# rustic-rs/rustic_core

Measured on AMD Instinct MI355X. Metric: CDC chunking GiB/s device-resident, 1/2/4/8 MI355X; bit-exact cut points vs ref, higher is better.
Workload: dtype u8

## Files before the change

rustic_core_amd/csrc/rcdc_ingest.cpp:

```cpp
#include <hip/hip_runtime.h>

#include <sys/random.h>

#include <algorithm>
#include <atomic>
#include <chrono>
#include <cmath>
#include <condition_variable>
#include <cstdio>
#include <cstdlib>
#include <cstring>
#include <deque>
#include <functional>
#include <memory>
#include <mutex>
#include <string>
#include <thread>
#include <unordered_map>
#include <unordered_set>
#include <vector>

#include "../../include/rcdc.h"
#include "rcdc_host.h"
#include "rcdc_ingest_steps.h"
// ... 33 lines not shown
    }
};

template <typename H, hipError_t (*Destroy)(H)>
struct HipOwner {
    H h = nullptr;
    HipOwner() = default;
    HipOwner(HipOwner &&o) noexcept : h(o.h) { o.h = nullptr; }
    ~HipOwner() { reset(); }
    void reset() {
        if (h) (void)Destroy(h);
        h = nullptr;
    }
    operator H() const { return h; }
};
using Stream = HipOwner<hipStream_t, hipStreamDestroy>;
struct Event : HipOwner<hipEvent_t, hipEventDestroy> {
    hipError_t create() { return hipEventCreateWithFlags(&h, hipEventDisableTiming); }
};

hipError_t ing_alloc(rcdc_ingest *g, void **p, uint64_t n, bool pinned);
hipError_t ing_free(void *p);

template <typename T>
struct IngBuf {
    T *p = nullptr;
    uint64_t cap = 0;
    bool pinned = false;
    IngBuf() = default;
    IngBuf(const IngBuf &) = delete;
    ~IngBuf() { (void)release(); }
    operator T *() const { return p; }
    hipError_t release() {
        T *q = p;
        p = nullptr, cap = 0;
        return q ? ing_free(q) : hipSuccess;
    }
    hipError_t alloc(rcdc_ingest *g, uint64_t n, bool pin) {
        pinned = pin;
        const hipError_t e = ing_alloc(g, (void **)&p, n * sizeof(T), pin);
        cap = e == hipSuccess ? n : 0;
        return e;
    }
    bool ensure(rcdc_ingest *g, uint64_t need, uint64_t grown, const char *what);
};

struct StreamSt {
    uint64_t handle = 0, tag = 0, hint = 0;
    uint64_t fed = 0;
    uint32_t open_pieces = 0;
    bool closed = false, aborted = false;
    int cslot = -1;
    uint64_t base = 0;
    uint64_t carry_len = 0;
    std::vector<uint8_t> hcarry;
    std::vector<uint64_t> cuts;
    std::vector<uint8_t> ids;
    uint32_t nnew = 0;
};

struct FileEnt {
    uint64_t tag = 0;
    uint64_t off = 0;
    uint64_t res = 0;
    uint64_t len = 0;
    bool done = false;
    bool cancelled = false;
    bool final = false;
    std::shared_ptr<StreamSt> st;
};

struct Unit {
    uint64_t tag = 0;
    std::shared_ptr<StreamSt> st;
    bool final = true, aborted = false;
    uint64_t base = 0;
    uint64_t carry = 0;
    uint64_t off = 0, len = 0;
    uint64_t fresh = 0;
    std::vector<std::pair<uint64_t, uint64_t>> segs;
    std::vector<std::pair<const uint8_t *, uint64_t>> host;
};

enum SlotState { kFree = 0, kOpen, kClosed, kSubmitted };

struct InSlot {
    IngBuf<uint8_t> host;
    uint64_t used = 0;
    uint32_t open_res = 0;
    SlotState state = kFree;
    std::vector<FileEnt> files;
    Event h2d;
    bool h2d_pending = false;
    std::atomic<int> host_jobs{0};
    std::atomic<bool> h2d_issued{false};
    uint64_t close_seq = 0;
    bool has_stream = false;
    double t_first = 0;
    void reset(SlotState to) {
        state = to;
        used = 0;
        files.clear();
        has_stream = false;
        t_first = 0;
    }
};

struct OutSlot {
    IngBuf<uint8_t> host;
    std::atomic<int> packs_left{0};
    bool busy = false;
};

struct D2HDone {
    Event fin;
    std::atomic<bool> issued{false};
};

struct Batch {
    uint64_t index = 0;
    uint32_t pslot = 0;
    InSlot *in = nullptr;
    std::vector<FileEnt> files;
    std::vector<Unit> units;
    std::vector<uint64_t> cuts;
    std::vector<uint32_t> ncuts;
    std::vector<uint64_t> c_off, c_len;
    std::vector<const uint8_t *> c_host;
    std::vector<std::vector<uint8_t>> gathers;
    std::vector<uint8_t> ids;
    std::vector<uint32_t> short_idx;
    std::vector<uint64_t> seal_off, seal_len, ulen;
    std::atomic<int> long_jobs{0};
    std::vector<rcdc_pack_blob> blobs;
    std::vector<std::pair<uint32_t, uint32_t>> grp;
    size_t open_from = 0;
    std::vector<rcdc_pack> packs;
    uint64_t total = 0;
    std::vector<uint32_t> boffs;
    OutSlot *out = nullptr;
    std::vector<std::pair<steps::D2HRange, std::shared_ptr<D2HDone>>> d2h;
};

struct PlanDel {
    void operator()(rcdc_plan *p) const { rcdc_plan_destroy(p); }
};
struct PSlot {
    std::unique_ptr<rcdc_plan, PlanDel> plan;
    IngBuf<uint8_t> arena;
    IngBuf<uint8_t> staging;
    IngBuf<uint64_t> d_refs;
    IngBuf<uint64_t> h_refs;
    IngBuf<uint8_t> d_dig;
    Stream s_ids;
    Event ev_ids;
    Event ev_sealed;
    Event ev_retired;
    bool busy = false;
};

struct PackJob {
    OutSlot *out = nullptr;
    uint64_t off = 0, size = 0, seq = 0, batch = 0;
    uint32_t header_len = 0;
    std::vector<rcdc_ingest_blob> blobs;
    uint8_t id[32];
};

long long env_num(const char *name, long long dflt) {
    const char *e = getenv(name);
    return e ? strtoll(e, nullptr, 10) : dflt;
}
struct Knobs {
    size_t tail_batches = (size_t)env_num("RCDC_INGEST_TAIL_BATCHES", 2);
    uint64_t d2h_group = (uint64_t)env_num("RCDC_INGEST_D2H_GROUP", 256ll << 20);
    bool tail_single = env_num("RCDC_INGEST_TAIL_SINGLE", 1) != 0;
    uint32_t id_threads = (uint32_t)env_num("RCDC_INGEST_ID_THREADS", 0);
    bool poll = env_num("RCDC_INGEST_POLL", 1) != 0;
    uint32_t kcopy = (uint32_t)std::max(env_num("RCDC_INGEST_KCOPY", 0), 0ll);
    uint64_t copy_piece = (uint64_t)std::max(env_num("RCDC_INGEST_COPY_PIECE", 64ll << 20), 1ll << 20);
    int prof = getenv("RCDC_INGEST_PROF") ? (int)std::max(env_num("RCDC_INGEST_PROF", 0), 1ll) : 0;
    uint32_t fail_alloc = (uint32_t)std::max(env_num("RCDC_INGEST_FAIL_ALLOC", 0), 0ll);
    bool alloc_log = getenv("RCDC_ALLOC_LOG") != nullptr;
};

}

struct rcdc_index {
    static constexpr int kShards = 64;
    struct Shard {
        std::mutex mu;
        std::unordered_set<Id32, Id32Hash> set;
    };
    Shard sh[kShards];
    bool insert(const Id32 &id) {
        Shard &s = sh[id.b[31] & (kShards - 1)];
        std::lock_guard<std::mutex> lk(s.mu);
        return s.set.insert(id).second;
    }
    uint64_t size() {
        uint64_t n = 0;
        for (auto &s : sh) {
            std::lock_guard<std::mutex> lk(s.mu);
            n += s.set.size();
        }
        return n;
    }
};

struct rcdc_ingest {
    rcdc_ctx *ctx = nullptr;
    rcdc_ingest_config cfg{};
    rcdc_ingest_pack_fn pack_cb = nullptr;
    rcdc_ingest_file_fn file_cb = nullptr;
    void *user = nullptr;
    int device = 0;
    int level = 0;
    bool compress = true, verify = true;
    uint64_t batch_cap = 0, long_chunk = 0;
    Knobs knobs;
    uint32_t depth = 4, nin = 4, nout = 4, nthreads = 8;
    PackSizer sizer{};
    std::mutex mu;
    std::condition_variable cv_slot;
    std::vector<std::unique_ptr<InSlot>> in;
    InSlot *open = nullptr;
    std::deque<InSlot *> ready;
    std::vector<PSlot> ps;
    IngBuf<uint8_t> frames;
    IngBuf<uint8_t> d_packs;
    IngBuf<uint8_t> carry[2];
    int carry_cur = 0;
    std::vector<rcdc_pack_blob> carry_blobs;
    Stream s_in, s_comp, s_out;
    Event ev_comp, ev_out, ev_back;
    std::vector<std::unique_ptr<OutSlot>> outs;
    std::deque<std::unique_ptr<Batch>> submitted;
    std::deque<std::unique_ptr<Batch>> inflight;
    bool front_done = false;
    uint64_t nclosed = 0;
    Stream s_back;
    uint64_t nbatches = 0, next_seq = 0;
    rcdc_index *idx = nullptr;
    std::unique_ptr<rcdc_index> own_idx;
    uint64_t max_chunk = 0;
    uint64_t asm_base = 0, asm_cap = 0;
    IngBuf<uint8_t> carry_pool;
    std::vector<int> free_cslots;
    std::unordered_map<uint64_t, std::shared_ptr<StreamSt>> streams;
    uint64_t next_stream = 1;
    uint32_t closing_streams = 0;
    std::deque<InSlot *> closed_q;
    double pack_t0 = 0;
    double pack_max_age = 300, slot_max_age = 1;
    uint32_t nalloc = 0;
    std::thread worker, back, waiter, feeder;
    struct CopyJob {
        uint8_t *dst;
        const uint8_t *src;
        uint64_t len, done;
        InSlot *in;
        Event after;
        std::shared_ptr<D2HDone> fin;
    };
    std::deque<CopyJob> h2d_q;
    std::mutex d2h_mu;
    std::deque<CopyJob> d2h_q;
    std::shared_ptr<D2HDone> last_d2h;
    int submitting = 0;
    std::vector<std::thread> pool;
    std::mutex pool_mu;
    std::condition_variable pool_cv;
    std::deque<std::function<void()>> jobs;
    std::deque<std::function<void()>> ujobs;
    uint32_t running_packs = 0;
    std::mutex wait_mu;
    std::condition_variable wait_cv;
    struct WaitItem {
        std::shared_ptr<D2HDone> done;
        uint64_t batch;
        std::vector<std::shared_ptr<PackJob>> jobs;
    };
    std::deque<WaitItem> wait_q;
    std::mutex cb_mu;
    std::atomic<bool> stop{false};
    bool finishing = false, finished = false;
    std::atomic<int> packs_pending{0};
    std::condition_variable cv_done;
    rcdc_status err = RCDC_OK;
    std::string err_msg;
    rcdc_ingest_stats st{};
    double t_first = 0;
    std::vector<std::vector<double>> tl;
    std::vector<double> tl_d2h, tl_ids;
};

namespace {

using Ing = rcdc_ingest;

void set_err(Ing *g, rcdc_status s, const std::string &m) {
    std::lock_guard<std::mutex> lk(g->mu);
    if (!g->err) {
        g->err = s;
        g->err_msg = m;
    }
    g->cv_slot.notify_all();
    g->cv_done.notify_all();
}

// ... 177 lines not shown
            std::vector<uint8_t> dig(32 * grp.size());
            for (auto &pj : grp) {
                ptrs.push_back(pj->out->host + pj->off);
                lens.push_back(pj->size);
            }
            hash_group(ptrs.data(), lens.data(), (uint32_t)grp.size(), dig.data(), mb);
            for (size_t i = 0; i < grp.size(); i++) {
                memcpy(grp[i]->id, dig.data() + 32 * i, 32);
                deliver(g, grp[i]);
            }
        });
    }
}

void waiter_main(Ing *g) {
    (void)hipSetDevice(g->device);
    for (;;) {
        Ing::WaitItem w;
        {
            std::unique_lock<std::mutex> lk(g->wait_mu);
            g->wait_cv.wait(lk, [&] { return g->stop || !g->wait_q.empty(); });
            if (g->wait_q.empty()) return;
            w = std::move(g->wait_q.front());
            g->wait_q.pop_front();
        }
        while (!w.done->issued.load() && !g->err && !g->stop)
            std::this_thread::sleep_for(std::chrono::microseconds(50));
        if (!w.done->issued.load()) continue;
        if (wait_event(g, w.done->fin) != hipSuccess) {
            set_err(g, RCDC_ERR_INTERNAL, "pack copy-back failed");
            continue;
        }
        if (g->knobs.prof) {
            std::lock_guard<std::mutex> lk(g->cb_mu);
            if (g->tl_d2h.size() <= w.batch) g->tl_d2h.resize(w.batch + 1, 0);
            g->tl_d2h[w.batch] = now_s() - g->t_first;
        }
        bool is_last;
        {
            std::lock_guard<std::mutex> lk(g->mu);
            is_last = g->front_done && g->inflight.size() <= 2;
            if (!is_last && g->finishing && g->ready.size() + g->nbatches <= w.batch + 4)
                is_last = true;
        }
        hash_packs(g, std::move(w.jobs), is_last);
    }
}

void mark(Ing *g, uint64_t b, double t) {
    if (!g->knobs.prof) return;
    std::lock_guard<std::mutex> lk(g->cb_mu);
    if (g->tl.size() <= b) g->tl.resize(b + 1);
    g->tl[b].push_back(t - g->t_first);
}

bool submit_ready(Ing *g) {
    for (;;) {
        InSlot *in = nullptr;
        uint32_t ps = 0;
        std::unique_ptr<Batch> B;
        {
            std::lock_guard<std::mutex> lk(g->mu);
            if (g->ready.empty()) return true;
            for (ps = 0; ps < g->depth && g->ps[ps].busy; ps++) {
            }
            if (ps == g->depth) return true;
            in = g->ready.front();
            g->ready.pop_front();
            g->submitting++;
            g->ps[ps].busy = true;
            B = std::make_unique<Batch>();
            B->index = g->nbatches++;
            if (g->t_first == 0) g->t_first = now_s();
        }
        B->pslot = ps;
        B->in = in;
        B->files = in->files;
        mark(g, B->index, now_s());
        PSlot &P = g->ps[ps];
        const uint64_t used = in->used;
        const uint64_t need = round_up(used, 256) + 512;
        if (!P.arena.ensure(g, need, grow8(need), "arena")) return false;
        in->h2d_issued = false;
        g->h2d_q.push_back({P.arena, in->host, used, 0, in, {}, nullptr});
        std::lock_guard<std::mutex> lk(g->mu);
        g->submitted.push_back(std::move(B));
        g->submitting--;
        g->cv_slot.notify_all();
    }
}

void reap_inputs(Ing *g);
void close_open_locked(Ing *g);

struct CopyLane {
    std::deque<Event> inflight;
    std::vector<Event> free_ev;
    hipError_t create() {
        free_ev.resize(4);
        for (Event &e : free_ev)
            if (hipError_t r = e.create()) return r;
        return hipSuccess;
    }
};

template <typename Done>
bool pump(Ing *g, hipStream_t s, std::deque<Ing::CopyJob> &q, std::mutex *mu, hipMemcpyKind kind,
          CopyLane &L, Done on_done) {
    while (!L.inflight.empty() && hipEventQuery(L.inflight.front()) == hipSuccess) {
        L.free_ev.push_back(std::move(L.inflight.front()));
        L.inflight.pop_front();
    }
    std::unique_lock<std::mutex> lq;
    if (mu) lq = std::unique_lock<std::mutex>(*mu);
    while (!q.empty() && L.inflight.size() < 2 && !L.free_ev.empty()) {
        Ing::CopyJob &J = q.front();
        if (J.after) {
            ING_HIP(g, hipStreamWaitEvent(s, J.after, 0));
            J.after.reset();
        }
        const uint64_t n = std::min(g->knobs.copy_piece, J.len - J.done);
        if (n) {
            if (g->knobs.kcopy)
                ING_HIP(g, launch_stream_copy(J.dst + J.done, J.src + J.done, (n + 15) & ~15ull,
                                              g->knobs.kcopy, s));
            else
                ING_HIP(g, hipMemcpyAsync(J.dst + J.done, J.src + J.done, n, kind, s));
            ING_HIP(g, hipEventRecord(L.free_ev.back(), s));
            L.inflight.push_back(std::move(L.free_ev.back()));
            L.free_ev.pop_back();
            J.done += n;
        }
        if (J.done == J.len) {
            if (!on_done(J)) return false;
            q.pop_front();
        }
    }
    return true;
}

bool pump_h2d(Ing *g, CopyLane &L) {
    return pump(g, g->s_in, g->h2d_q, nullptr, hipMemcpyHostToDevice, L, [g](Ing::CopyJob &J) {
        ING_HIP(g, hipEventRecord(J.in->h2d, g->s_in));
        J.in->h2d_issued = true;
        std::lock_guard<std::mutex> lk(g->mu);
        g->cv_slot.notify_all();
        return true;
    });
}

bool pump_d2h(Ing *g, CopyLane &L) {
    return pump(g, g->s_out, g->d2h_q, &g->d2h_mu, hipMemcpyDeviceToHost, L, [g](Ing::CopyJob &J) {
        ING_HIP(g, hipEventRecord(g->ev_out, g->s_out));
        ING_HIP(g, hipEventRecord(J.fin->fin, g->s_out));
        J.fin->issued.store(true);
        return true;
    });
}

void feeder_main(Ing *g) {
    (void)hipSetDevice(g->device);
    CopyLane in, out;
    if (in.create() != hipSuccess || out.create() != hipSuccess) {
        set_err(g, RCDC_ERR_INTERNAL, "feeder events");
        return;
    }
    struct Drain {
        Ing *g;
        ~Drain() {
            (void)hipStreamSynchronize(g->s_in);
            (void)hipStreamSynchronize(g->s_out);
        }
    } drain{g};
    for (;;) {
        reap_inputs(g);
        if (!submit_ready(g) || !pump_h2d(g, in) || !pump_d2h(g, out)) return;
        bool d2h_idle;
        {
            std::lock_guard<std::mutex> lq(g->d2h_mu);
            d2h_idle = g->d2h_q.empty();
        }
        std::unique_lock<std::mutex> lk(g->mu);
        if (g->open && !g->open->files.empty() && now_s() - g->open->t_first >= g->slot_max_age)
            close_open_locked(g);
        if (g->err || (g->finished && g->h2d_q.empty() && d2h_idle)) return;
        g->cv_slot.wait_for(lk, std::chrono::microseconds(g->h2d_q.empty() && d2h_idle ? 200 : 50));
    }
}

const uint8_t *unit_host(const Unit &u, uint64_t rel, uint64_t len) {
    uint64_t at = 0;
    for (const auto &h : u.host) {
        if (rel >= at && rel + len <= at + h.second) return h.first + (rel - at);
        at += h.second;
    }
    return nullptr;
}

void unit_gather(const Unit &u, uint64_t rel, uint64_t len, uint8_t *dst) {
    uint64_t at = 0;
    for (const auto &h : u.host) {
        const uint64_t a = std::max(rel, at), e = std::min(rel + len, at + h.second);
        if (a < e) memcpy(dst + (a - rel), h.first + (a - at), e - a);
        at += h.second;
    }
}

bool build_units(Ing *g, Batch *B, std::vector<rcdc_copy_ref> &cr, uint64_t *asm_used) {
    InSlot *in = B->in;
    std::unordered_map<StreamSt *, size_t> unit_of;
    for (const FileEnt &f : B->files) {
        if (f.cancelled) continue;
        if (!f.st) {
            Unit u;
            u.tag = f.tag;
            u.off = f.off;
            u.len = u.fresh = f.len;
            u.segs.push_back({f.off, f.len});
            B->units.push_back(std::move(u));
            continue;
        }
        auto it = unit_of.find(f.st.get());
        if (it == unit_of.end()) {
            Unit u;
            u.st = f.st;
            u.tag = f.st->tag;
            u.final = false;
            u.base = f.st->base;
            u.carry = f.st->carry_len;
            it = unit_of.emplace(f.st.get(), B->units.size()).first;
            B->units.push_back(std::move(u));
        }
        Unit &u = B->units[it->second];
        if (f.final) {
            u.final = true;
            u.aborted = f.st->aborted;
        }
        if (!f.len) continue;
        if (!u.segs.empty() && u.segs.back().first + u.segs.back().second == f.off)
            u.segs.back().second += f.len;
        else
            u.segs.push_back({f.off, f.len});
        u.fresh += f.len;
    }
    uint64_t ao = 0;
    for (Unit &u : B->units) {
        if (!u.st) {
            u.host.push_back({in->host + u.off, u.len});
            continue;
        }
        u.len = u.carry + u.fresh;
        if (!u.carry && u.segs.size() <= 1) {
            u.off = u.segs.empty() ? 0 : u.segs[0].first;
            if (u.fresh) u.host.push_back({in->host + u.off, u.fresh});
            continue;
        }
        u.off = g->asm_base + ao;
        uint64_t o = u.off;
        if (u.carry) {
            rcdc_copy_ref c{};
            c.in_off = (uint64_t)u.st->cslot * g->max_chunk;
            c.out_off = o;
            c.len = u.carry;
            c.src = 1;
            cr.push_back(c);
            u.host.push_back({u.st->hcarry.data(), u.carry});
            o += u.carry;
        }
        for (const auto &sg : u.segs) {
            rcdc_copy_ref c{};
            c.in_off = sg.first;
            c.out_off = o;
            c.len = sg.second;
            c.src = 0;
            cr.push_back(c);
            u.host.push_back({in->host + sg.first, sg.second});
            o += sg.second;
        }
        ao = round_up(ao + u.len, 256);
        if (ao > g->asm_cap) {
            set_err(g, RCDC_ERR_INTERNAL, "ingest: assembly region overflow");
            return false;
        }
    }
    *asm_used = ao;
    return true;
}


bool a_wait_h2d(Ing *g, Batch *B) {
    InSlot *in = B->in;
    {
        std::unique_lock<std::mutex> lk(g->mu);
        while (!in->h2d_issued && !g->err) g->cv_slot.wait_for(lk, std::chrono::microseconds(100));
        if (g->err) return false;
    }
    ING_HIP(g, hipStreamWaitEvent(g->s_comp, in->h2d, 0));
    if (g->knobs.prof > 1) mark(g, B->index, now_s());
    return true;
}

bool a_gather_units(Ing *g, Batch *B, PSlot &P, uint64_t *arena_len) {
    std::vector<rcdc_copy_ref> gcr;
    uint64_t asm_used = 0;
    if (!build_units(g, B, gcr, &asm_used)) return false;
    if (!gcr.empty()) {
        const void *gsrc[2] = {P.arena, g->carry_pool};
        ING_ST(g, rcdc_copy_ranges(g->ctx, gsrc, 2, gcr.data(), (uint32_t)gcr.size(), P.arena,
                                   g->s_comp),
               "stream gather");
    }
    *arena_len = std::max(round_up(B->in->used, 256) + 256,
                          asm_used ? g->asm_base + asm_used + 256 : 0);
    return true;
}

bool a_chunk(Ing *g, Batch *B, PSlot &P, uint64_t arena_len, std::vector<uint64_t> &cuts,
             std::vector<uint64_t> &counts) {
    const uint32_t nf = (uint32_t)B->units.size();
    std::vector<uint64_t> offs(nf), lens(nf);
    uint64_t ubytes = 0;
    for (uint32_t i = 0; i < nf; i++) {
        offs[i] = B->units[i].off;
        lens[i] = B->units[i].len;
        ubytes += lens[i];
    }
    if (!P.plan) {
        rcdc_plan *pl = nullptr;
        ING_ST(g, rcdc_plan_create(g->ctx, offs.data(), lens.data(), nf, arena_len, &pl), "plan");
        P.plan.reset(pl);
    } else {
        ING_ST(g, plan_relayout(P.plan.get(), offs.data(), lens.data(), nf, arena_len, g->s_comp),
               "plan");
    }
    if (g->knobs.prof > 1) mark(g, B->index, now_s());
    ING_ST(g, rcdc_plan_run(P.plan.get(), P.arena, g->s_comp), "chunk");
    if (g->knobs.prof > 1) {
        (void)hipEventSynchronize(B->in->h2d);
        mark(g, B->index, now_s());
    }
    const uint64_t cap = (uint64_t)nf + ubytes / 4096 + 16;
    cuts.assign(std::max<uint64_t>(cap, 1), 0);
    counts.assign(std::max<uint32_t>(nf, 1), 0);
    rcdc_status rs = rcdc_plan_results(P.plan.get(), cuts.data(), cuts.size(), counts.data());
    if (rs == RCDC_ERR_CAPACITY) {
        uint64_t tot = 0;
        for (uint32_t i = 0; i < nf; i++) tot += counts[i];
        cuts.resize(tot);
        rs = rcdc_plan_results(P.plan.get(), cuts.data(), cuts.size(), counts.data());
    }
    ING_ST(g, rs, "chunk results");
    mark(g, B->index, now_s());
    return true;
}

steps::CutLists a_cut_lists(Ing *g, Batch *B, const std::vector<uint64_t> &cuts,
                            const std::vector<uint64_t> &counts) {
    std::vector<steps::UnitView> uv;
    for (const Unit &u : B->units)
// ... 432 lines not shown

void b_post_packs(Ing *g, Batch *B) {
    std::vector<std::shared_ptr<PackJob>> jobs;
    for (size_t j = 0; j < B->grp.size(); j++) {
        auto pj = std::make_shared<PackJob>();
        pj->out = B->out;
        pj->off = B->packs[j].out_off;
        pj->size = B->packs[j].size;
        pj->header_len = B->packs[j].header_len;
        pj->seq = g->next_seq++;
        pj->batch = B->index;
        for (uint32_t i = B->grp[j].first; i < B->grp[j].first + B->grp[j].second; i++) {
            rcdc_ingest_blob e{};
            memcpy(e.id, B->blobs[i].id, 32);
            e.offset = B->boffs[i];
            e.length = B->blobs[i].len;
            e.uncompressed_length = B->blobs[i].uncompressed_len;
            e.type = B->blobs[i].type;
            pj->blobs.push_back(e);
        }
        jobs.push_back(pj);
    }
    B->out->packs_left += (int)jobs.size();
    g->packs_pending += (int)jobs.size();
    {
        std::lock_guard<std::mutex> lk(g->mu);
        g->st.packs += jobs.size();
        g->st.pack_bytes += B->total;
    }
    {
        std::lock_guard<std::mutex> lk(g->wait_mu);
        for (auto &d : B->d2h)
            g->wait_q.push_back({d.second, B->index,
                                 std::vector<std::shared_ptr<PackJob>>(
                                     jobs.begin() + d.first.first, jobs.begin() + d.first.last)});
    }
    g->wait_cv.notify_one();
}

bool stage_b(Ing *g, Batch *B, bool finalize) {
    const bool has_slot = B->pslot != kNoSlot;
    PSlot &P = g->ps[has_slot ? B->pslot : 0];
    mark(g, B->index, now_s());
    if (has_slot) {
        ING_HIP(g, wait_event(g, P.ev_ids));
        ING_HIP(g, hipStreamWaitEvent(g->s_back, P.ev_sealed, 0));
    }
    mark(g, B->index, now_s());
    if (!b_read_ids(g, B, P)) return false;
    std::vector<uint8_t> is_new;
    const size_t nnew = b_dedup(g, B, is_new);
    b_file_results(g, B, is_new);
    const double tnow = now_s();
    const bool carried = !g->carry_blobs.empty();
    const bool aged = carried && tnow - g->pack_t0 >= g->pack_max_age;
    B->grp = steps::group_packs(B->blobs.data(), B->blobs.size(), g->sizer, finalize, aged,
                                &B->open_from);
    B->packs.assign(B->grp.size(), rcdc_pack{});
    B->total = steps::layout_packs(B->blobs.data(), B->grp, B->packs.data());
    std::vector<uint8_t> hn(16 * B->grp.size());
    random_bytes(hn.data(), hn.size());
    for (size_t j = 0; j < B->grp.size(); j++) memcpy(B->packs[j].header_nonce, hn.data() + 16 * j, 16);
    if (!B->grp.empty() && (!b_build_packs(g, B) || !b_queue_d2h(g, B, finalize))) return false;
    if (!b_carry_open_pack(g, B, carried, tnow)) return false;
    if (!B->grp.empty()) b_post_packs(g, B);
    if (has_slot) ING_HIP(g, hipEventRecord(P.ev_retired, g->s_back));
    {
        std::lock_guard<std::mutex> lk(g->mu);
        g->st.new_blobs += nnew;
    }
    mark(g, B->index, now_s());
    return true;
}

bool close_open_pack(Ing *g) {
    Batch empty;
    empty.pslot = kNoSlot;
    empty.index = g->nbatches;
    return stage_b(g, &empty, true);
}

void reap_inputs(Ing *g) {
    std::lock_guard<std::mutex> lk(g->mu);
    for (auto &s : g->in)
        if (s->state == kSubmitted && s->host_jobs == 0 &&
            (!s->h2d_pending || hipEventQuery(s->h2d) == hipSuccess)) {
            s->h2d_pending = false;
            s->reset(kFree);
            g->cv_slot.notify_all();
        }
}

void worker_main(Ing *g) {
    (void)hipSetDevice(g->device);
    for (;;) {
        std::unique_ptr<Batch> B;
        bool done = false;
        {
            std::unique_lock<std::mutex> lk(g->mu);
            if (g->err) {
                g->cv_done.notify_all();
                return;
            }
            if (!g->submitted.empty()) {
                B = std::move(g->submitted.front());
                g->submitted.pop_front();
            } else {
                done = g->finishing && g->ready.empty() && g->open == nullptr &&
                       g->closed_q.empty() && g->submitting == 0;
            }
        }
        if (B) {
            if (!stage_a(g, B.get())) return;
            std::lock_guard<std::mutex> lk(g->mu);
            g->inflight.push_back(std::move(B));
            g->cv_slot.notify_all();
            continue;
        }
        std::unique_lock<std::mutex> lk(g->mu);
        if (done) {
            g->front_done = true;
            g->cv_slot.notify_all();
            return;
        }
        g->cv_slot.wait_for(lk, std::chrono::microseconds(200));
    }
}

void back_main(Ing *g) {
    (void)hipSetDevice(g->device);
    for (;;) {
        std::unique_ptr<Batch> B;
        bool last = false, all_done = false, fin_carry = false, aged = false;
        {
            std::unique_lock<std::mutex> lk(g->mu);
            for (;;) {
                if (g->err) {
                    g->cv_done.notify_all();
                    return;
                }
                if (!g->inflight.empty() && g->inflight.front()->long_jobs == 0) break;
                if (g->inflight.empty() && g->front_done) break;
                if (g->inflight.empty() && !g->carry_blobs.empty() &&
                    now_s() - g->pack_t0 >= g->pack_max_age) {
                    aged = true;
                    break;
                }
                g->cv_slot.wait_for(lk, std::chrono::microseconds(200));
            }
            if (aged) {
            } else if (!g->inflight.empty()) {
                B = std::move(g->inflight.front());
                g->inflight.pop_front();
                last = g->front_done && g->inflight.empty();
            } else {
                all_done = true;
                fin_carry = !g->carry_blobs.empty();
            }
        }
        if (aged) {
            if (!close_open_pack(g)) return;
            continue;
        }
        if (B) {
            if (!stage_b(g, B.get(), last)) return;
            std::lock_guard<std::mutex> lk(g->mu);
            g->ps[B->pslot].busy = false;
            g->cv_slot.notify_all();
            continue;
        }
        if (all_done) {
            if (fin_carry && !close_open_pack(g)) return;
            std::unique_lock<std::mutex> lk(g->mu);
            g->finished = true;
            g->cv_done.notify_all();
            return;
        }
    }
}

void promote_locked(Ing *g) {
    bool head = true;
    for (auto it = g->closed_q.begin(); it != g->closed_q.end();) {
        InSlot *s = *it;
        if (s->open_res == 0 && (head || !s->has_stream)) {
            it = g->closed_q.erase(it);
            bool empty = true;
            for (const FileEnt &f : s->files) empty &= f.cancelled;
            if (empty) {
                s->reset(kFree);
            } else {
                g->ready.push_back(s);
            }
            g->cv_slot.notify_all();
            continue;
        }
        head = false;
        ++it;
    }
}

void close_open_locked(Ing *g) {
    InSlot *s = g->open;
    if (!s) return;
    g->open = nullptr;
    s->close_seq = g->nclosed++;
    s->state = kClosed;
    g->closed_q.push_back(s);
    promote_locked(g);
    g->cv_slot.notify_all();
}

rcdc_status reserve_locked(Ing *g, std::unique_lock<std::mutex> &lk, uint64_t len,
                           const std::shared_ptr<StreamSt> &st, bool final, uint8_t **buf,
                           uint64_t *ticket) {
    for (;;) {
        if (g->err) return set_error(g->err, g->err_msg.c_str());
        if (g->finishing) return set_error(RCDC_ERR_INVALID_INPUT, "ingest already finishing");
        InSlot *s = g->open;
        const uint64_t cap_now = g->nclosed == 0 ? std::max(g->batch_cap / 4, len)
                                                 : (s ? s->host.cap : 0);
        uint64_t place = s ? s->used : 0;
        if (s && st && !s->files.empty()) {
            const FileEnt &b = s->files.back();
            if (b.st == st && b.done && !b.cancelled && s->used == round_up(b.off + b.res, 256))
                place = b.off + b.len;
        }
        if (s && place + len > cap_now) {
            close_open_locked(g);
            s = nullptr;
            place = 0;
        }
        if (!s) {
            for (auto &x : g->in)
                if (x->state == kFree) {
                    s = x.get();
                    break;
                }
            if (s) {
                s->reset(kOpen);
                g->open = s;
            }
        }
        if (s) {
            FileEnt f;
            f.off = place;
            f.res = len;
            f.st = st;
            f.final = final;
            s->files.push_back(f);
            s->used = round_up(place + len, 256);
            s->open_res++;
            s->has_stream |= st != nullptr;
            if (s->files.size() == 1) s->t_first = now_s();
            size_t idx = 0;
            for (; idx < g->in.size(); idx++)
                if (g->in[idx].get() == s) break;
            *ticket = ((uint64_t)idx << 32) | (uint64_t)(s->files.size() - 1);
            *buf = s->host + place;
            return RCDC_OK;
        }
        g->cv_slot.wait_for(lk, std::chrono::milliseconds(1));
        lk.unlock();
        reap_inputs(g);
        lk.lock();
    }
}

rcdc_status commit_locked(Ing *g, uint64_t ticket, uint64_t tag, uint64_t len, bool cancel) {
    const uint64_t si = ticket >> 32, fi = ticket & 0xFFFFFFFFull;
    if (si >= g->in.size() || fi >= g->in[si]->files.size() || g->in[si]->files[fi].done ||
        (g->in[si]->state != kOpen && g->in[si]->state != kClosed))
        return set_error(RCDC_ERR_INVALID_INPUT, "bad ticket");
    InSlot *s = g->in[si].get();
    FileEnt &f = s->files[fi];
    if (len > f.res) return set_error(RCDC_ERR_INVALID_INPUT, "commit longer than the reservation");
    if (!f.st) f.tag = tag;
    f.len = cancel ? 0 : len;
    f.done = true;
    f.cancelled = cancel;
    if (f.st) {
        f.st->fed += f.len;
        f.st->open_pieces--;
    }
    s->open_res--;
    if (s->state == kClosed && s->open_res == 0) promote_locked(g);
    return RCDC_OK;
}

std::shared_ptr<StreamSt> find_stream(Ing *g, uint64_t h) {
    auto it = g->streams.find(h);
    return it == g->streams.end() ? nullptr : it->second;
}

rcdc_status stream_end(Ing *g, uint64_t handle, bool abort) {
    if (!g) return set_error(RCDC_ERR_INVALID_INPUT, "null argument");
    std::unique_lock<std::mutex> lk(g->mu);
    auto st = find_stream(g, handle);
    if (!st) return set_error(RCDC_ERR_INVALID_INPUT, "unknown stream");
    if (st->open_pieces)
        return set_error(RCDC_ERR_INVALID_INPUT, "stream has pieces not committed or cancelled");
    uint8_t *buf;
    uint64_t t;
    if (rcdc_status rs = reserve_locked(g, lk, 0, st, true, &buf, &t)) return rs;
    st->closed = true;
    st->aborted = abort;
    g->streams.erase(handle);
    g->closing_streams++;
    return commit_locked(g, t, 0, 0, false);
}

struct Sizes {
    uint64_t batch_cap, max_chunk, min_chunk;
    uint32_t depth, nin, nout, nthreads, max_streams;
    uint64_t out_slot, asm_base, asm_cap, arena, staging, refs_cap, frames, carry, carry_pool;
    uint64_t pinned() const { return nin * batch_cap + nout * out_slot + depth * refs_cap * 16; }
    uint64_t device() const {
        return depth * (arena + staging + refs_cap * 48) + 2 * frames + 2 * carry + carry_pool;
    }
};

Sizes engine_sizes(const rcdc_ctx *ctx, const rcdc_ingest_config *cfg, uint64_t pack_size) {
    Sizes z{};
    z.batch_cap = round_up(cfg->batch_bytes ? cfg->batch_bytes : (2ull << 30), 256);
    z.max_chunk = round_up(std::max<uint64_t>(ctx_max_size(ctx), 64), 256);
    z.min_chunk = std::max<uint64_t>(ctx_min_size(ctx), 4096);
    z.depth = cfg->depth ? cfg->depth : 4;
    z.nin = std::max(cfg->in_slots ? cfg->in_slots : 4u, 2u);
    z.nout = std::max(cfg->out_slots ? cfg->out_slots : 4u, 1u);
    z.nthreads = cfg->hash_threads ? cfg->hash_threads : 10;
    z.max_streams = cfg->max_streams ? cfg->max_streams : 16;
    z.out_slot = z.batch_cap + z.batch_cap / 16 + (64ull << 20);
    z.asm_base = round_up(z.batch_cap + 1024, 256);
    z.asm_cap = z.batch_cap + (uint64_t)z.max_streams * (z.max_chunk + 256) + 256;
    z.arena = z.asm_base + z.asm_cap + 1024;
    const uint64_t chunked = z.batch_cap + (uint64_t)z.max_streams * z.max_chunk;
    z.staging = chunked + chunked / 64 + (64ull << 20);
    z.frames = z.staging;
    z.refs_cap = chunked / z.min_chunk * 2 + 1024;
    z.carry = std::max<uint64_t>(pack_size * 2, 128ull << 20);
    z.carry_pool = (uint64_t)z.max_streams * z.max_chunk;
    return z;
}

rcdc_status create_fail(hipError_t e, const char *what) {
    return set_error(RCDC_ERR_INTERNAL, (std::string(what) + ": " + hipGetErrorString(e)).c_str());
}
#define NEW_TRY(expr, what)                                         \
    do {                                                            \
        hipError_t e_ = (expr);                                     \
        if (e_ != hipSuccess) return create_fail(e_, what);         \
    } while (0)

rcdc_status build_pslot(Ing *g, PSlot &P, const Sizes &z) {
    int prio_lo = 0, prio_hi = 0;
    (void)hipDeviceGetStreamPriorityRange(&prio_lo, &prio_hi);
    NEW_TRY(hipStreamCreateWithPriority(&P.s_ids.h, hipStreamNonBlocking, prio_lo), "stream");
    NEW_TRY(P.ev_ids.create(), "stream");
    NEW_TRY(P.ev_sealed.create(), "stream");
    NEW_TRY(P.ev_retired.create(), "stream");
    NEW_TRY(P.arena.alloc(g, z.arena, false), "arena");
    NEW_TRY(P.staging.alloc(g, z.staging, false), "staging");
    constexpr uint32_t kPlanStreams = 256;
    std::vector<uint64_t> off0(kPlanStreams), len0(kPlanStreams);
    const uint64_t per = (g->batch_cap / kPlanStreams) & ~255ull;
    for (uint32_t i = 0; i < kPlanStreams; i++) {
        off0[i] = i * per;
        len0[i] = per;
    }
    rcdc_plan *pl = nullptr;
    if (rcdc_status ps = rcdc_plan_create(g->ctx, off0.data(), len0.data(), kPlanStreams,
                                          g->batch_cap + 256, &pl))
        return ps;
    P.plan.reset(pl);
    std::vector<uint64_t> wc(g->batch_cap / 4096 + kPlanStreams + 16), wn(kPlanStreams);
    for (uint32_t ns : {0u, 1u, 2u, 4u, 16u}) {
        std::vector<uint64_t> o(ns), l(ns);
        const uint64_t each = (g->batch_cap / std::max(ns, 1u)) & ~255ull;
        for (uint32_t i = 0; i < ns; i++) {
            o[i] = i * each;
            l[i] = each;
        }
        if (rcdc_status ps = ns ? rcdc::plan_relayout(pl, o.data(), l.data(), ns,
                                                      g->batch_cap + 256, nullptr)
                                : RCDC_OK)
            return ps;
        if (rcdc_status ps = rcdc_plan_run(pl, P.arena, nullptr)) return ps;
        if (rcdc_status ps = rcdc_plan_results(pl, wc.data(), wc.size(), wn.data());
            ps && ps != RCDC_ERR_CAPACITY)
            return ps;
    }
    NEW_TRY(P.h_refs.alloc(g, z.refs_cap * 2, true), "refs");
    NEW_TRY(P.d_refs.alloc(g, z.refs_cap * 2, false), "refs");
    NEW_TRY(P.d_dig.alloc(g, z.refs_cap * 32, false), "refs");
    return RCDC_OK;
}

rcdc_status build_engine(Ing *g, const Sizes &z) {
    for (uint32_t i = 0; i < g->nin; i++) {
        g->in.push_back(std::make_unique<InSlot>());
        NEW_TRY(g->in.back()->host.alloc(g, g->batch_cap, true), "input slot");
        NEW_TRY(g->in.back()->h2d.create(), "event");
    }
    for (uint32_t i = 0; i < g->nout; i++) {
        g->outs.push_back(std::make_unique<OutSlot>());
        NEW_TRY(g->outs.back()->host.alloc(g, z.out_slot, true), "output slot");
    }
    for (int c = 0; c < 2; c++) NEW_TRY(g->carry[c].alloc(g, z.carry, false), "carry");
    NEW_TRY(g->carry_pool.alloc(g, z.carry_pool, false), "stream carries");
    g->ps = std::vector<PSlot>(g->depth);
    for (auto &P : g->ps)
        if (rcdc_status st = build_pslot(g, P, z)) return st;
    NEW_TRY(g->frames.alloc(g, z.frames, false), "frames");
    NEW_TRY(g->d_packs.alloc(g, z.frames, false), "packs");
    NEW_TRY(hipStreamCreateWithFlags(&g->s_in.h, hipStreamNonBlocking), "streams");
    NEW_TRY(hipStreamCreateWithFlags(&g->s_comp.h, hipStreamNonBlocking), "streams");
    NEW_TRY(hipStreamCreateWithFlags(&g->s_out.h, hipStreamNonBlocking), "streams");
    NEW_TRY(hipStreamCreateWithFlags(&g->s_back.h, hipStreamNonBlocking), "streams");
    NEW_TRY(g->ev_comp.create(), "streams");
    NEW_TRY(g->ev_back.create(), "streams");
    NEW_TRY(g->ev_out.create(), "streams");
    NEW_TRY(hipEventRecord(g->ev_out, g->s_out), "event");
    return RCDC_OK;
}
#undef NEW_TRY

}

extern "C" {

void rcdc_ingest_config_default(rcdc_ingest_config *c) {
    if (!c) return;
    memset(c, 0, sizeof *c);
    c->zstd_level = 0;
    c->compress = 1;
    c->extra_verify = 1;
    c->pack_size = 32ull << 20;
    c->pack_grow_factor = 32;
    c->pack_size_limit = 0xFFFFFFFFull;
    c->batch_bytes = 2ull << 30;
    c->depth = 4;
    c->in_slots = 4;
    c->out_slots = 4;
    c->hash_threads = 10;
    c->max_streams = 16;
    c->long_chunk = 2ull << 20;
    c->pack_max_age_ms = 300000;
    c->slot_max_age_ms = 1000;
}

rcdc_status rcdc_ingest_footprint(const rcdc_ctx *ctx, const rcdc_ingest_config *cfg,
                                  uint64_t *pinned, uint64_t *device) {
    if (!ctx || !cfg) return set_error(RCDC_ERR_INVALID_INPUT, "null argument");
    PackSizer ps{cfg->pack_size ? cfg->pack_size : (32ull << 20), cfg->pack_grow_factor,
                 cfg->pack_size_limit ? cfg->pack_size_limit : 0xFFFFFFFFull, cfg->pack_current_size};
    const Sizes z = engine_sizes(ctx, cfg, ps.pack_size());
    if (pinned) *pinned = z.pinned();
    if (device) *device = z.device();
    return RCDC_OK;
}

void rcdc_ingest_mem_live(uint64_t *pinned, uint64_t *device) {
    std::lock_guard<std::mutex> lk(g_alloc_mu);
    if (pinned) *pinned = g_live_pinned;
    if (device) *device = g_live_dev;
}

rcdc_status rcdc_ingest_create(rcdc_ctx *ctx, const rcdc_ingest_config *cfg,
                               rcdc_ingest_pack_fn pack_cb, rcdc_ingest_file_fn file_cb,
                               void *user, rcdc_ingest **out) {
    if (!ctx || !cfg || !out) return set_error(RCDC_ERR_INVALID_INPUT, "null argument");
    if (cfg->zstd_level < -131072 || cfg->zstd_level > 22)
        return set_error(RCDC_ERR_INVALID_INPUT, "zstd level out of range");
    auto g = std::make_unique<rcdc_ingest>();
    g->ctx = ctx;
    g->cfg = *cfg;
    g->pack_cb = pack_cb;
    g->file_cb = file_cb;
    g->user = user;
    g->device = ctx_device(ctx);
    g->level = cfg->zstd_level;
    g->compress = cfg->compress != 0;
    g->verify = cfg->extra_verify != 0;
    g->sizer.default_size = cfg->pack_size ? cfg->pack_size : (32ull << 20);
    g->sizer.grow = cfg->pack_grow_factor;
    g->sizer.limit = cfg->pack_size_limit ? cfg->pack_size_limit : 0xFFFFFFFFull;
    g->sizer.current = cfg->pack_current_size;
    const Sizes z = engine_sizes(ctx, cfg, g->sizer.pack_size());
    g->batch_cap = z.batch_cap;
    g->long_chunk = cfg->long_chunk ? cfg->long_chunk : (2ull << 20);
    g->depth = z.depth;
    g->nin = z.nin;
    g->nout = z.nout;
    g->nthreads = z.nthreads;
    g->max_chunk = z.max_chunk;
    g->asm_base = z.asm_base;
    g->asm_cap = z.asm_cap;
    g->pack_max_age = (cfg->pack_max_age_ms ? cfg->pack_max_age_ms : 300000) / 1e3;
    g->slot_max_age = (cfg->slot_max_age_ms ? cfg->slot_max_age_ms : 1000) / 1e3;
    g->own_idx = std::make_unique<rcdc_index>();
    g->idx = g->own_idx.get();
    for (uint32_t i = 0; i < z.max_streams; i++) g->free_cslots.push_back((int)(z.max_streams - 1 - i));
    Ing *gp = g.get();
    (void)hipSetDevice(g->device);
    if (rcdc_status st = build_engine(gp, z)) {
        const std::string m = rcdc_last_error();
        g.reset();
        return set_error(st, m.c_str());
    }
    for (uint32_t i = 0; i < g->nthreads; i++) g->pool.emplace_back(pool_main, gp);
    g->waiter = std::thread(waiter_main, gp);
    g->worker = std::thread(worker_main, gp);
    g->feeder = std::thread(feeder_main, gp);
    g->back = std::thread(back_main, gp);
    *out = g.release();
    return RCDC_OK;
}

rcdc_status rcdc_ingest_add_index(rcdc_ingest *g, const uint8_t *ids, uint64_t n) {
    if (!g || (n && !ids)) return set_error(RCDC_ERR_INVALID_INPUT, "null argument");
    std::lock_guard<std::mutex> lk(g->mu);
    if (g->nbatches) return set_error(RCDC_ERR_INVALID_INPUT, "index ids after the first batch");
    return rcdc_index_add(g->idx, ids, n);
}

rcdc_status rcdc_ingest_reserve(rcdc_ingest *g, uint64_t len, uint8_t **buf, uint64_t *ticket) {
    if (!g || !buf || !ticket) return set_error(RCDC_ERR_INVALID_INPUT, "null argument");
    if (len > g->batch_cap)
        return set_error(RCDC_ERR_UNSUPPORTED,
                         "file larger than the ingest batch (batch_bytes): feed it as a stream "
                         "(rcdc_ingest_stream_open)");
    std::unique_lock<std::mutex> lk(g->mu);
    return reserve_locked(g, lk, len, nullptr, false, buf, ticket);
}

rcdc_status rcdc_ingest_commit(rcdc_ingest *g, uint64_t ticket, uint64_t tag, uint64_t len) {
    if (!g) return set_error(RCDC_ERR_INVALID_INPUT, "null argument");
    std::lock_guard<std::mutex> lk(g->mu);
    return commit_locked(g, ticket, tag, len, false);
}

rcdc_status rcdc_ingest_cancel(rcdc_ingest *g, uint64_t ticket) {
    if (!g) return set_error(RCDC_ERR_INVALID_INPUT, "null argument");
    std::lock_guard<std::mutex> lk(g->mu);
    return commit_locked(g, ticket, 0, 0, true);
}

rcdc_status rcdc_ingest_stream_open(rcdc_ingest *g, uint64_t tag, uint64_t size_hint,
                                    uint64_t *stream) {
    if (!g || !stream) return set_error(RCDC_ERR_INVALID_INPUT, "null argument");
    std::unique_lock<std::mutex> lk(g->mu);
    for (;;) {
        if (g->err) return set_error(g->err, g->err_msg.c_str());
        if (g->finishing) return set_error(RCDC_ERR_INVALID_INPUT, "ingest already finishing");
        if (!g->free_cslots.empty()) break;
        if (!g->closing_streams)
            return set_error(RCDC_ERR_UNSUPPORTED, "max_streams streams are open");
        close_open_locked(g);
        g->cv_slot.wait_for(lk, std::chrono::milliseconds(1));
    }
    auto st = std::make_shared<StreamSt>();
    st->handle = g->next_stream++;
    st->tag = tag;
    st->hint = size_hint;
    st->cslot = g->free_cslots.back();
    g->free_cslots.pop_back();
    g->streams[st->handle] = st;
    *stream = st->handle;
    return RCDC_OK;
}

rcdc_status rcdc_ingest_stream_reserve(rcdc_ingest *g, uint64_t stream, uint64_t len,
// ... 173 lines not shown
```

rustic_core_amd/csrc/rcdc_ingest_steps.h:

```cpp
#pragma once

#include <algorithm>
#include <cmath>
#include <cstddef>
#include <cstdint>
#include <utility>
#include <vector>

#include "../../include/rcdc.h"

namespace rcdc {
namespace steps {

constexpr uint64_t kMaxPackSize = 4076ull << 20;
constexpr uint32_t kMaxPackCount = 10000;

struct PackSizer {
    uint64_t default_size, grow, limit, current;
    uint64_t pack_size() const {
        uint64_t size = default_size;
        if (grow) size = ((uint64_t)std::sqrt((double)current) * grow + default_size) & 0xFFFFFFFFull;
        return std::min(std::min(size, limit), kMaxPackSize);
    }
};

inline uint64_t header_entry_len(const rcdc_pack_blob &b) { return b.uncompressed_len ? 41 : 37; }

inline std::vector<std::pair<uint32_t, uint32_t>> group_packs(const rcdc_pack_blob *blobs,
                                                              size_t n, PackSizer &sizer,
                                                              bool finalize, bool aged,
                                                              size_t *open_from) {
    std::vector<std::pair<uint32_t, uint32_t>> grp;
    size_t b0 = 0;
    while (b0 < n) {
        const uint64_t limit = sizer.pack_size();
        uint64_t sz = 0, hdr = 0;
        size_t e = b0;
        while (e < n && sz < limit && e - b0 < kMaxPackCount) {
            sz += blobs[e].len;
            hdr += header_entry_len(blobs[e]);
            e++;
        }
        const bool closed = sz >= limit || e - b0 >= kMaxPackCount;
        if (!closed && !finalize && !(aged && b0 == 0)) break;
        grp.push_back({(uint32_t)b0, (uint32_t)(e - b0)});
        sizer.current += sz + hdr + 32 + 4;
        b0 = e;
    }
    *open_from = b0;
    return grp;
}

inline uint64_t layout_packs(const rcdc_pack_blob *blobs,
                             const std::vector<std::pair<uint32_t, uint32_t>> &grp,
                             rcdc_pack *packs) {
    uint64_t total = 0;
    for (size_t j = 0; j < grp.size(); j++) {
        uint64_t sz = 32 + 4;
        for (uint32_t i = grp[j].first; i < grp[j].first + grp[j].second; i++)
            sz += blobs[i].len + header_entry_len(blobs[i]);
        packs[j].out_off = total;
        packs[j].blob0 = grp[j].first;
        packs[j].nblobs = grp[j].second;
        total += sz;
    }
    return total;
}

struct D2HRange {
    size_t first, last;
    uint64_t lo, hi;
};
inline std::vector<D2HRange> d2h_ranges(const rcdc_pack *packs, size_t n, uint64_t total,
                                        uint64_t group_bytes) {
    std::vector<D2HRange> out;
    for (size_t a = 0; a < n;) {
        size_t b = a + 1;
        while (b < n && packs[b].out_off - packs[a].out_off < group_bytes) b++;
        out.push_back({a, b, packs[a].out_off, b < n ? packs[b].out_off : total});
        a = b;
    }
    return out;
}

struct UnitView {
    bool stream, final, aborted;
    uint64_t off, len;
    int cslot;
};
struct CutLists {
    std::vector<uint64_t> cuts;
    std::vector<uint32_t> ncuts;
    std::vector<uint64_t> c_off, c_len;
    std::vector<std::pair<uint32_t, uint64_t>> carries;
    std::vector<rcdc_copy_ref> copies;
};
inline CutLists cut_lists(const std::vector<UnitView> &units, const uint64_t *counts,
                          const uint64_t *cuts, uint64_t max_chunk) {
    CutLists L;
    L.ncuts.resize(units.size());
    uint64_t k = 0;
    for (size_t i = 0; i < units.size(); i++) {
        const UnitView &u = units[i];
        const uint64_t n = counts[i];
        uint64_t keep = n;
        if (u.stream && (!u.final || u.aborted)) {
            keep = n ? n - 1 : 0;
            const uint64_t from = keep ? cuts[k + keep - 1] : 0;
            if (!u.aborted) {
                L.carries.push_back({(uint32_t)i, from});
                if (u.len > from) {
                    rcdc_copy_ref c{};
                    c.in_off = u.off + from;
                    c.out_off = (uint64_t)u.cslot * max_chunk;
                    c.len = u.len - from;
                    c.src = 0;
                    L.copies.push_back(c);
                }
            }
        }
        L.ncuts[i] = (uint32_t)keep;
        uint64_t prev = 0;
        for (uint64_t j = 0; j < keep; j++) {
            L.cuts.push_back(cuts[k + j]);
            L.c_off.push_back(u.off + prev);
            L.c_len.push_back(cuts[k + j] - prev);
            prev = cuts[k + j];
        }
        k += n;
    }
    return L;
}

}
}
```

Measured before the change: 7824.

## Ramp batch sizes at ingest start and split tail batches into views

Adds a geometric batch-size ramp: the first batches close at a fraction of batch_cap and double each time, so the GPU pipeline starts sooner. At finish, remaining ready slots are split into smaller sub-slot views at file boundaries, sized to shrink the pipeline drain tail. Views share the parent host memory and the parent is freed when all its views are reaped. Plan warmup is also run for the ramp sizes. This adds more small batches and more per-batch overhead, along with extra lifetime-tracking complexity.

```diff
diff --git a/rustic_core_amd/csrc/rcdc_ingest.cpp b/rustic_core_amd/csrc/rcdc_ingest.cpp
--- a/rustic_core_amd/csrc/rcdc_ingest.cpp
+++ b/rustic_core_amd/csrc/rcdc_ingest.cpp
@@ -139,10 +139,13 @@
     std::vector<std::pair<const uint8_t *, uint64_t>> host;
 };
 
-enum SlotState { kFree = 0, kOpen, kClosed, kSubmitted };
+enum SlotState { kFree = 0, kOpen, kClosed, kSubmitted, kSplit };
 
 struct InSlot {
     IngBuf<uint8_t> host;
+    uint8_t *mem = nullptr;
+    InSlot *parent = nullptr;
+    uint32_t views = 0;
     uint64_t used = 0;
     uint32_t open_res = 0;
     SlotState state = kFree;
@@ -239,6 +242,10 @@
     int prof = getenv("RCDC_INGEST_PROF") ? (int)std::max(env_num("RCDC_INGEST_PROF", 0), 1ll) : 0;
     uint32_t fail_alloc = (uint32_t)std::max(env_num("RCDC_INGEST_FAIL_ALLOC", 0), 0ll);
     bool alloc_log = getenv("RCDC_ALLOC_LOG") != nullptr;
+    uint32_t ramp = ramp_div(env_num("RCDC_INGEST_RAMP", 1));
+    static uint32_t ramp_div(long long v) {
+        return v <= 0 ? 0u : v == 1 ? 8u : (uint32_t)std::min(v, 1ll << 20);
+    }
 };
 
 }
@@ -283,6 +290,9 @@
     std::vector<std::unique_ptr<InSlot>> in;
     InSlot *open = nullptr;
     std::deque<InSlot *> ready;
+    steps::Ramp ramp{};
+    std::vector<std::unique_ptr<InSlot>> views;
+    bool tail_split_done = false;
     std::vector<PSlot> ps;
     IngBuf<uint8_t> frames;
     IngBuf<uint8_t> d_packs;
@@ -626,7 +636,7 @@
         const uint64_t need = round_up(used, 256) + 512;
         if (!P.arena.ensure(g, need, grow8(need), "arena")) return false;
         in->h2d_issued = false;
-        g->h2d_q.push_back({P.arena, in->host, used, 0, in, {}, nullptr});
+        g->h2d_q.push_back({P.arena, in->mem, used, 0, in, {}, nullptr});
         std::lock_guard<std::mutex> lk(g->mu);
         g->submitted.push_back(std::move(B));
         g->submitting--;
@@ -636,6 +646,65 @@
 
 void reap_inputs(Ing *g);
 void close_open_locked(Ing *g);
+
+void split_tail(Ing *g) {
+    std::lock_guard<std::mutex> lk(g->mu);
+    if (!g->finishing || g->tail_split_done || g->err) return;
+    if (g->open || !g->closed_q.empty()) return;
+    g->tail_split_done = true;
+    if (!g->ramp.start_div) return;
+    uint64_t left = 0;
+    for (InSlot *s : g->ready) left += s->used;
+    std::deque<InSlot *> out;
+    for (InSlot *s : g->ready) {
+        std::vector<size_t> first{0};
+        uint64_t base = 0, target = steps::tail_target(g->ramp, left);
+        for (size_t i = 1; i < s->files.size(); i++) {
+            const uint64_t off = s->files[i].off;
+            if (off % 256 || !target || off - base < target) continue;
+            left -= off - base;
+            base = off;
+            target = steps::tail_target(g->ramp, left);
+            first.push_back(i);
+        }
+        left -= s->used - base;
+        std::vector<std::unique_ptr<InSlot>> vs;
+        bool ok = first.size() > 1;
+        for (size_t k = 0; k < first.size() && ok; k++) {
+            const bool last = k + 1 == first.size();
+            const size_t a = first[k], b = last ? s->files.size() : first[k + 1];
+            const uint64_t lo = s->files[a].off, hi = last ? s->used : s->files[b].off;
+            auto v = std::make_unique<InSlot>();
+            v->mem = s->mem + lo;
+            v->parent = s;
+            v->used = hi - lo;
+            v->state = kClosed;
+            v->close_seq = s->close_seq;
+            bool empty = true;
+            for (size_t i = a; i < b; i++) {
+                FileEnt f = s->files[i];
+                f.off -= lo;
+                empty &= f.cancelled;
+                v->has_stream |= f.st != nullptr;
+                v->files.push_back(std::move(f));
+            }
+            if (empty) continue;
+            ok = v->h2d.create() == hipSuccess;
+            vs.push_back(std::move(v));
+        }
+        if (!ok || vs.empty()) {
+            out.push_back(s);
+            continue;
+        }
+        s->state = kSplit;
+        s->views = (uint32_t)vs.size();
+        for (auto &v : vs) {
+            out.push_back(v.get());
+            g->views.push_back(std::move(v));
+        }
+    }
+    g->ready.swap(out);
+}
 
 struct CopyLane {
     std::deque<Event> inflight;
@@ -718,6 +787,7 @@
     } drain{g};
     for (;;) {
         reap_inputs(g);
+        split_tail(g);
         if (!submit_ready(g) || !pump_h2d(g, in) || !pump_d2h(g, out)) return;
         bool d2h_idle;
         {
@@ -790,13 +860,13 @@
     uint64_t ao = 0;
     for (Unit &u : B->units) {
         if (!u.st) {
-            u.host.push_back({in->host + u.off, u.len});
+            u.host.push_back({in->mem + u.off, u.len});
             continue;
         }
         u.len = u.carry + u.fresh;
         if (!u.carry && u.segs.size() <= 1) {
             u.off = u.segs.empty() ? 0 : u.segs[0].first;
-            if (u.fresh) u.host.push_back({in->host + u.off, u.fresh});
+            if (u.fresh) u.host.push_back({in->mem + u.off, u.fresh});
             continue;
         }
         u.off = g->asm_base + ao;
@@ -818,7 +888,7 @@
             c.len = sg.second;
             c.src = 0;
             cr.push_back(c);
-            u.host.push_back({in->host + sg.first, sg.second});
+            u.host.push_back({in->mem + sg.first, sg.second});
             o += sg.second;
         }
         ao = round_up(ao + u.len, 256);
@@ -1417,13 +1487,15 @@
 
 void reap_inputs(Ing *g) {
     std::lock_guard<std::mutex> lk(g->mu);
-    for (auto &s : g->in)
-        if (s->state == kSubmitted && s->host_jobs == 0 &&
-            (!s->h2d_pending || hipEventQuery(s->h2d) == hipSuccess)) {
-            s->h2d_pending = false;
-            s->reset(kFree);
-            g->cv_slot.notify_all();
-        }
+    for (auto *slots : {&g->in, &g->views})
+        for (auto &s : *slots)
+            if (s->state == kSubmitted && s->host_jobs == 0 &&
+                (!s->h2d_pending || hipEventQuery(s->h2d) == hipSuccess)) {
+                s->h2d_pending = false;
+                s->reset(kFree);
+                if (s->parent && --s->parent->views == 0) s->parent->reset(kFree);
+                g->cv_slot.notify_all();
+            }
 }
 
 void worker_main(Ing *g) {
@@ -1553,8 +1625,10 @@
         if (g->err) return set_error(g->err, g->err_msg.c_str());
         if (g->finishing) return set_error(RCDC_ERR_INVALID_INPUT, "ingest already finishing");
         InSlot *s = g->open;
-        const uint64_t cap_now = g->nclosed == 0 ? std::max(g->batch_cap / 4, len)
-                                                 : (s ? s->host.cap : 0);
+        const uint64_t thr = g->ramp.start_div ? steps::ramp_threshold(g->ramp, g->nclosed)
+                             : g->nclosed == 0 ? g->batch_cap / 4
+                                               : g->batch_cap;
+        const uint64_t cap_now = std::max(thr, len);
         uint64_t place = s ? s->used : 0;
         if (s && st && !s->files.empty()) {
             const FileEnt &b = s->files.back();
@@ -1593,6 +1667,10 @@
                 if (g->in[idx].get() == s) break;
             *ticket = ((uint64_t)idx << 32) | (uint64_t)(s->files.size() - 1);
             *buf = s->host + place;
+            if (g->ramp.start_div) {
+                const uint64_t t = steps::ramp_threshold(g->ramp, g->nclosed);
+                if (t < g->batch_cap && s->used >= t) close_open_locked(g);
+            }
             return RCDC_OK;
         }
         g->cv_slot.wait_for(lk, std::chrono::milliseconds(1));
@@ -1725,6 +1803,22 @@
             ps && ps != RCDC_ERR_CAPACITY)
             return ps;
     }
+    for (uint64_t b = 0; steps::ramp_threshold(g->ramp, b) < g->batch_cap; b++) {
+        const uint64_t sz = steps::ramp_threshold(g->ramp, b);
+        for (uint32_t ns : {1u, 4u}) {
+            const uint64_t each = (sz / ns) & ~255ull;
+            if (!each) continue;
+            std::vector<uint64_t> o(ns), l(ns, each);
+            for (uint32_t i = 0; i < ns; i++) o[i] = i * each;
+            if (rcdc_status ps = rcdc::plan_relayout(pl, o.data(), l.data(), ns,
+                                                     round_up(sz, 256) + 256, nullptr))
+                return ps;
+            if (rcdc_status ps = rcdc_plan_run(pl, P.arena, nullptr)) return ps;
+            if (rcdc_status ps = rcdc_plan_results(pl, wc.data(), wc.size(), wn.data());
+                ps && ps != RCDC_ERR_CAPACITY)
+                return ps;
+        }
+    }
     NEW_TRY(P.h_refs.alloc(g, z.refs_cap * 2, true), "refs");
     NEW_TRY(P.d_refs.alloc(g, z.refs_cap * 2, false), "refs");
     NEW_TRY(P.d_dig.alloc(g, z.refs_cap * 32, false), "refs");
@@ -1735,6 +1829,7 @@
     for (uint32_t i = 0; i < g->nin; i++) {
         g->in.push_back(std::make_unique<InSlot>());
         NEW_TRY(g->in.back()->host.alloc(g, g->batch_cap, true), "input slot");
+        g->in.back()->mem = g->in.back()->host;
         NEW_TRY(g->in.back()->h2d.create(), "event");
     }
     for (uint32_t i = 0; i < g->nout; i++) {
@@ -1823,6 +1918,7 @@
     g->sizer.current = cfg->pack_current_size;
     const Sizes z = engine_sizes(ctx, cfg, g->sizer.pack_size());
     g->batch_cap = z.batch_cap;
+    g->ramp = {z.batch_cap, g->knobs.ramp};
     g->long_chunk = cfg->long_chunk ? cfg->long_chunk : (2ull << 20);
     g->depth = z.depth;
     g->nin = z.nin;
diff --git a/rustic_core_amd/csrc/rcdc_ingest_steps.h b/rustic_core_amd/csrc/rcdc_ingest_steps.h
--- a/rustic_core_amd/csrc/rcdc_ingest_steps.h
+++ b/rustic_core_amd/csrc/rcdc_ingest_steps.h
@@ -83,6 +83,30 @@
     return out;
 }
 
+struct Ramp {
+    uint64_t batch_bytes;
+    uint32_t start_div;
+    uint64_t floor() const {
+        return start_div ? std::max<uint64_t>(batch_bytes / start_div, 1) : batch_bytes;
+    }
+};
+inline uint64_t ramp_threshold(const Ramp &r, uint64_t index) {
+    uint64_t t = r.floor();
+    for (uint64_t i = 0; i < index && t < r.batch_bytes; i++) t *= 2;
+    return std::min(t, r.batch_bytes);
+}
+inline uint64_t tail_target(const Ramp &r, uint64_t left) {
+    return std::min(std::min(left, r.batch_bytes), std::max(r.floor(), left - left / 2));
+}
+inline std::vector<uint64_t> tail_split(const Ramp &r, uint64_t left) {
+    std::vector<uint64_t> out;
+    while (left) {
+        out.push_back(tail_target(r, left));
+        left -= out.back();
+    }
+    return out;
+}
+
 struct UnitView {
     bool stream, final, aborted;
     uint64_t off, len;
```

After: 7824, median of 2. Within noise of the previous version (-0.0%).
